# yassine-cherni/mujoco_ros2_simulation

Hardware: AMD Instinct MI355X
Metric: env-steps/sec (whole node), 7-DoF arm+lidar scene at 1/2/4/8 MI355X (higher is better)
Workload: dtype f32

## Files before the change

### include/mrs.h

```cpp
#ifndef MRS_H
#define MRS_H

#include "mrs_model.h"

#ifdef __cplusplus
extern "C" {
#endif

typedef struct mrs_model mrs_model;
typedef struct mrs_batch mrs_batch;

enum {
  MRS_OK = 0,
  MRS_ERR_INVALID = -1,
  MRS_ERR_LOAD = -2,
  MRS_ERR_DEVICE = -3,
  MRS_ERR_UNSUPPORTED = -4
};

enum {
  MRS_FIELD_QPOS = 0,
  MRS_FIELD_QVEL = 1,
  MRS_FIELD_CTRL = 2,
  MRS_FIELD_QFRC_APPLIED = 3,
// ... 101 lines not shown
int mrs_batch_get_contact_forces(mrs_batch* b, int env, int max, double* force);
float* mrs_batch_contact_wrench_device_ptr(mrs_batch* b);
int mrs_batch_get_contact_wrench(mrs_batch* b, double* host, int env0, int n);
enum {
  MRS_DYNOUT_QFRC_BIAS = 0,
  MRS_DYNOUT_MASS_MATRIX = 1,
  MRS_DYNOUT_SITE_JAC = 2,
  MRS_DYNOUT_SITE_POSE = 3,
  MRS_DYNOUT_COUNT = 4
};
#define MRS_MAX_JAC_SITES 16
int mrs_batch_set_jac_sites(mrs_batch* b, const int* site_ids, int n);
int mrs_batch_dyn_dim(const mrs_batch* b, int which);
float* mrs_batch_dyn_device_ptr(mrs_batch* b, int which);
int mrs_batch_get_dyn(mrs_batch* b, int which, double* host, int env0, int n);
int mrs_batch_get_efc(mrs_batch* b, int env, int max, int* type, double* J, double* R, double* aref,
                      double* force);
int mrs_batch_get_field_device(mrs_batch* b, int field, float* d_out, int env0, int n);
int mrs_batch_sync(mrs_batch* b);
double mrs_batch_last_kernel_ms(mrs_batch* b, int kind);
int mrs_batch_set_timing(mrs_batch* b, int mask);
int mrs_debug_phase_cycles(double* out, int n, int reset);
int mrs_debug_batch_layout(const mrs_batch* b, int* out, int n);
int mrs_debug_plan_layout(const mrs_model* m, int n_envs, int cu_count, int max_contacts, int* out, int n);
int mrs_debug_render_plan(const mrs_model* m, int cam, int n_frames, int max_lds, long long* out, int n);
int mrs_debug_ray_filter(const mrs_model* m, unsigned group_mask, int flags, int bodyexclude, int* out, int max);

#ifdef __cplusplus
}
#endif
#endif
```

### mujoco_ros2_simulation_amd/csrc/capi.cc

```cpp
#include <algorithm>
#include <cstring>
#include <memory>
#include <stdexcept>
#include <string>
#include <vector>

#include "../../include/mrs.h"
#include "hip/batch.h"
#include "mjcf/model.h"
#include "hip/rayfilter.h"
#include "hip/start_rows.h"
#include "mjcf/xml.h"

struct mrs_model {
  mrs::Model m;
};
struct mrs_batch {
  mrs::BatchImpl* impl = nullptr;
  const mrs_model* model = nullptr;
};

namespace {

thread_local std::string g_last_error;
// ... 532 lines not shown
  return ms;
}

int mrs_debug_phase_cycles(double* out, int n, int reset) {
  if (!out || n < 0) return MRS_ERR_INVALID;
  return mrs::phase_cycles(out, n, reset != 0);
}

int mrs_debug_batch_layout(const mrs_batch* b, int* out, int n) {
  if (!b || !out || n < 0) return MRS_ERR_INVALID;
  return mrs::batch_layout(b->impl, out, n);
}

int mrs_debug_plan_layout(const mrs_model* m, int n_envs, int cu_count, int max_contacts, int* out, int n) {
  int k = 0;
  const int rc = guarded([&] {
    if (!m || !out || n < 0) throw std::invalid_argument("null model or output");
    if (n_envs < 1) throw std::invalid_argument("n_envs must be positive");
    k = mrs::plan_layout(m->m, n_envs, cu_count, max_contacts, out, n);
  });
  return rc == MRS_OK ? k : rc;
}

int mrs_debug_render_plan(const mrs_model* m, int cam, int n_frames, int max_lds, long long* out, int n) {
  int k = 0;
  const int rc = guarded([&] {
    if (!m || !out || n < 0) throw std::invalid_argument("null model or output");
    if (n_frames < 1) throw std::invalid_argument("n_frames must be positive");
    if (max_lds < 0) throw std::invalid_argument("negative LDS limit");
    k = mrs::render_plan(m->m, cam, n_frames, max_lds, out, n);
  });
  return rc == MRS_OK ? k : rc;
}

int mrs_debug_ray_filter(const mrs_model* m, unsigned group_mask, int flags, int bodyexclude, int* out, int max) {
  int k = 0;
  const int rc = guarded([&] {
    if (!m) throw std::invalid_argument("null model");
    if (max < 0 || (max > 0 && !out)) throw std::invalid_argument("null output or negative capacity");
    mrs::check_ray_filter(m->m, flags, bodyexclude);
    const std::vector<mrs::RayGeom> list =
        mrs::build_ray_filter(m->m, group_mask, (flags & MRS_RAY_NO_STATIC) != 0, bodyexclude);
    k = static_cast<int>(list.size());
    for (int i = 0; i < k && i < max; ++i) out[i] = list[i].id;
  });
  return rc == MRS_OK ? k : rc;
// ... 4 lines not shown
```

### mujoco_ros2_simulation_amd/csrc/hip/batch.h

```cpp
#pragma once

#include <stdexcept>
#include <string>

namespace mrs {

struct Model;
struct BatchImpl;

struct DeviceError : std::runtime_error { using std::runtime_error::runtime_error; };
struct UnsupportedError : std::runtime_error { using std::runtime_error::runtime_error; };

BatchImpl* batch_create(const Model* model, int n_envs, int device, int max_contacts);
void batch_free(BatchImpl* b);
int batch_num_envs(const BatchImpl* b);
int batch_layout(const BatchImpl* b, int* out, int n);
int plan_layout(const Model& m, int n_envs, int cu_count, int max_contacts, int* out, int n);
void batch_set_stream(BatchImpl* b, void* stream);
void batch_reset(BatchImpl* b, int key, int env0, int n);
void batch_set_start_states(BatchImpl* b, const double* qpos, const double* qvel, int count);
void batch_set_start_states_device(BatchImpl* b, const float* d_qpos, const float* d_qvel, int count);
int batch_num_start_states(const BatchImpl* b);
void batch_reset_masked_device(BatchImpl* b, const unsigned char* d_mask, const int* d_key, int key);
void batch_reset_masked(BatchImpl* b, const unsigned char* mask, const int* keys, int key);
void batch_set(BatchImpl* b, int field, const double* host, int env0, int n);
void batch_get(BatchImpl* b, int field, double* host, int env0, int n);
void* batch_device_ptr(BatchImpl* b, int field);
void batch_set_act(BatchImpl* b, const double* host, int env0, int n);
void batch_get_act(BatchImpl* b, double* host, int env0, int n);
float* batch_act_device_ptr(BatchImpl* b);
void batch_set_mocap(BatchImpl* b, const double* pos, const double* quat, int env0, int n);
void batch_get_mocap(BatchImpl* b, double* pos, double* quat, int env0, int n);
float* batch_mocap_pos_device_ptr(BatchImpl* b);
float* batch_mocap_quat_device_ptr(BatchImpl* b);
int batch_param_dim(BatchImpl* b, int param);
void batch_set_param(BatchImpl* b, int param, const double* host, int env0, int n);
void batch_get_param(BatchImpl* b, int param, double* host, int env0, int n);
float* batch_param_device_ptr(BatchImpl* b, int param);
int batch_inertial_dim(BatchImpl* b, int which);
void batch_set_inertial(BatchImpl* b, const double* mass, const double* inertia, const double* armature, int env0, int n);
// ... 31 lines not shown
```

### mujoco_ros2_simulation_amd/csrc/hip/batch.hip

```cpp
#include <hip/hip_runtime.h>

#include <algorithm>
#include <cmath>
#include <cstdio>
#include <cstdlib>
#include <cstring>
#include <deque>
#include <initializer_list>
#include <stdexcept>
#include <string>
#include <thread>
#include <type_traits>
#include <utility>
#include <vector>

#include "../../../include/mrs.h"
#include "../mjcf/model.h"
#include "batch.h"
#include "batch_impl.h"
#include "devmodel.h"
#include "devtables.h"
#include "plan.h"
#include "lit.h"
#include "start_rows.h"
// ... 150 lines not shown
    a.bind(dalloc(b, static_cast<size_t>(b.n) * std::max(1, a.dim) * a.width()));
  }
}

void build_devmodel(BatchImpl& b, int max_con_req, const Overrides& o) {
  const Model& m = *b.model;
  const DevTables T = build_tables(m, max_con_req, o);
  int cus = 0;
  if (hipDeviceGetAttribute(&cus, hipDeviceAttributeMultiprocessorCount, b.device) != hipSuccess) cus = 0;
  const Plan p = choose_plan(m, T, b.n, cus, o);
  void* made[kArrCount];
  for (int id = 0; id < kArrCount; ++id) made[id] = env_array(b, id).ptr;
  b.dm = p.dm;
  for (int id = 0; id < kArrCount; ++id)
    if (made[id]) env_array(b, id).bind(made[id]);
  b.dblock_f = dalloc(b, T.f.size() * sizeof(float));
  b.dblock_i = dalloc(b, T.i.size() * sizeof(int));
  HIP_CHECK(hipMemcpyAsync(b.dblock_f, T.f.data(), T.f.size() * sizeof(float), hipMemcpyHostToDevice, b.stream));
  HIP_CHECK(hipMemcpyAsync(b.dblock_i, T.i.data(), T.i.size() * sizeof(int), hipMemcpyHostToDevice, b.stream));
  T.patch(b.dm, static_cast<const float*>(b.dblock_f), static_cast<const int*>(b.dblock_i));
  b.dm.rf_static = b.dm.rf_mode ? static_cast<float*>(dalloc(b, std::max(1, b.dm.nrf) * sizeof(float))) : nullptr;
  b.group = p.group; b.g16_one_wg = p.g16_one_wg; b.wpb16 = p.wpb16; b.helpers = p.helpers; b.ext = p.ext;
  b.pair_g1 = T.pair_g1; b.pair_g2 = T.pair_g2; b.pair_dim = T.pair_dim; b.pair_mu = T.pair_mu;
  b.d_dm = static_cast<DevModel*>(dalloc(b, sizeof(DevModel)));
  HIP_CHECK(hipMemcpyAsync(b.d_dm, &b.dm, sizeof(DevModel), hipMemcpyHostToDevice, b.stream));
  HIP_CHECK(hipStreamSynchronize(b.stream));
}

struct RowStage { double* host; std::vector<float> f; std::vector<int> i; };

void rows_to_device(BatchImpl& b, int env0, int n, std::initializer_list<std::pair<EnvArray, const double*>> parts) {
  HIP_CHECK(hipSetDevice(b.device));
  std::deque<RowStage> stage;
  bool queued = false;
  for (const auto& part : parts) {
    const EnvArray& a = part.first;
    const double* host = part.second;
    const size_t cnt = static_cast<size_t>(n) * std::max(0, a.dim);
    if (!host || cnt == 0) continue;
    const void* src = host;
    if (a.type == EnvArray::F32) {
      std::vector<float>& t = stage.emplace_back().f;
      t.resize(cnt);
      for (size_t k = 0; k < cnt; ++k) t[k] = static_cast<float>(host[k]);
      src = t.data();
    } else if (a.type == EnvArray::I32) {
// ... 204 lines not shown
  return b;
}

void batch_free(BatchImpl* b) {
  if (!b) return;
  (void)hipSetDevice(b->device);
  if (b->stream) (void)hipStreamSynchronize(b->stream);
  if (b->rstream) (void)hipStreamSynchronize(b->rstream);
  for (void* p : b->allocs) (void)hipFree(p);
  if (b->pool_qpos) (void)hipFree(b->pool_qpos);
  if (b->pool_qvel) (void)hipFree(b->pool_qvel);
  render_free(*b);
  for (int k = 0; k < 2; ++k) {
    if (b->ev0[k]) (void)hipEventDestroy(b->ev0[k]);
    if (b->ev1[k]) (void)hipEventDestroy(b->ev1[k]);
  }
  if (b->own_stream) (void)hipStreamDestroy(b->own_stream);
  delete b;
}

int batch_num_envs(const BatchImpl* b) { return b->n; }

int batch_layout(const BatchImpl* b, int* out, int n) {
  int v[19];
  plan_layout_values(b->dm, b->group, b->g16_one_wg, b->wpb16, b->helpers, v);
  v[16] = b->dm.cfrc_contact ? 1 : 0;
  v[17] = b->dm.dyn_mask;
  v[18] = b->dm.solve_fuse;
  int k = 0;
  for (; k < n && k < 19; ++k) out[k] = v[k];
  return k;
}

int plan_layout(const Model& m, int n_envs, int cu_count, int max_contacts, int* out, int n) {
  const Overrides o = read_overrides();
  const DevTables T = build_tables(m, max_contacts, o);
  const Plan p = choose_plan(m, T, n_envs, cu_count, o);
  int v[kPlanLayoutValues];
  plan_layout_values(p.dm, p.group, p.g16_one_wg, p.wpb16, p.helpers, v);
  int k = 0;
  for (; k < n && k < kPlanLayoutValues; ++k) out[k] = v[k];
  return k;
}

void batch_set_stream(BatchImpl* b, void* stream) {
  b->stream = stream ? static_cast<hipStream_t>(stream) : b->own_stream;
}

void batch_reset(BatchImpl* b, int key, int env0, int n) {
  const Model& m = *b->model;
  check_env_range(*b, env0, n);
  if (key >= m.nkey) throw std::invalid_argument("keyframe index out of range");
  b->ctrl_bound = nullptr;
// ... 505 lines not shown
```

### mujoco_ros2_simulation_amd/csrc/hip/batch_impl.h

```cpp
#pragma once

#include <hip/hip_runtime.h>

#include <deque>
#include <stdexcept>
#include <string>
#include <vector>

#include "../mjcf/model.h"
#include "batch.h"
#include "devmodel.h"
#include "rayfilter.h"
#include "start_rows.h"

namespace mrs {

#define HIP_CHECK(x)                                                                         \
  do {                                                                                       \
    hipError_t err_ = (x);                                                                   \
    if (err_ != hipSuccess)                                                                  \
      throw DeviceError(std::string(#x) + " failed: " + hipGetErrorString(err_));            \
  } while (0)

struct BatchImpl {
// ... 7 lines not shown
  DevModel* d_dm = nullptr;
  LdsLayout& L = dm.L;
  ScratchLayout& S = dm.S;
  DevState st{};
  const float* ctrl_bound = nullptr;
  StartRows start;
  std::vector<double> inr_host;
  float *tab_qpos = nullptr, *tab_qvel = nullptr, *tab_ctrl = nullptr, *tab_act = nullptr;
  float *tab_mpos = nullptr, *tab_mquat = nullptr;
  double* tab_time = nullptr;
  float *pool_qpos = nullptr, *pool_qvel = nullptr;
  int pool_n = 0, pool_cap = 0;
  unsigned char* mask_stage = nullptr;
  int* key_stage = nullptr;
  void* dblock_f = nullptr;
  void* dblock_i = nullptr;
  std::vector<void*> allocs;
  hipStream_t own_stream = nullptr, stream = nullptr;
  hipEvent_t ev0[2] = {nullptr, nullptr}, ev1[2] = {nullptr, nullptr};
  bool ev_valid[2] = {false, false};
  int timing = 2;
  std::vector<float> staging;
  std::vector<int> pair_g1, pair_g2;
  std::vector<int> pair_dim;
  std::vector<float> pair_mu;
  int dyn_asked = 0;
  hipStream_t rstream = nullptr;
  hipEvent_t snap_ev = nullptr, rend_ev = nullptr;
  bool rend_pending = false;
  float *snap_gpos = nullptr, *snap_gmat = nullptr, *snap_cpos = nullptr, *snap_cmat = nullptr;
  unsigned long long* rast_list = nullptr;
  int rast_frames = 0;
  int max_lds = 0;
  struct RayList { unsigned group_mask; bool no_static; int bodyexclude; RayGeom* d; int count; bool mesh; };
  std::deque<RayList> ray_lists;
  bool ext = false;
};

inline void* dalloc(BatchImpl& b, size_t bytes) {
  void* p = nullptr;
  HIP_CHECK(hipMalloc(&p, bytes ? bytes : 16));
  HIP_CHECK(hipMemsetAsync(p, 0, bytes ? bytes : 16, b.stream));
  b.allocs.push_back(p);
  return p;
}

// ... 8 lines not shown
```

### mujoco_ros2_simulation_amd/csrc/hip/devtables.h

```cpp
#pragma once

#include <algorithm>
#include <array>
#include <cmath>
#include <cstdlib>
#include <cstring>
#include <functional>
#include <stdexcept>
#include <string>
#include <vector>

#include "../../../include/mrs.h"
#include "../mjcf/model.h"
#include "batch.h"
#include "devmodel.h"
#include "renderplan.h"
#include "start_rows.h"

namespace mrs {

struct Overrides {
  int group = 0;
  int g16_wpb = 0;
  bool g16_one_wg = false;
  bool ray_helpers = true;
  bool no_fuse_ih = false;
  bool no_solve_fuse = false;
  bool no_ray_sweep = false;
  bool no_static_rays = false;
  bool no_static_frame = false;
  bool kin_twopass = false;
  int sparse_off = 0;
  int diag_skip = 0;
  bool sensors_every_step = false;
  bool no_multiccd = false;
  bool no_bvh = false;
  int bvh_leaf = 4;
  bool bvh_median = false;
  int spread = 0;
};

inline Overrides read_overrides() {
  auto set = [](const char* name) { return std::getenv(name) != nullptr; };
  auto num = [](const char* name, int absent) { const char* e = std::getenv(name); return e ? std::atoi(e) : absent; };
  Overrides o;
  o.group = num("MRS_GROUP", 0);
  o.g16_wpb = num("MRS_G16_WPB", 0);
  o.g16_one_wg = set("MRS_G16_ONE_WG");
  o.ray_helpers = num("MRS_RAY_HELPERS", 1) != 0;
  o.no_fuse_ih = set("MRS_NO_FUSE_IH");
  o.no_solve_fuse = set("MRS_NO_SOLVE_FUSE");
  o.no_ray_sweep = set("MRS_NO_RAY_SWEEP");
  o.no_static_rays = set("MRS_NO_STATIC_RAYS");
  o.no_static_frame = set("MRS_NO_STATIC_FRAME");
  o.kin_twopass = set("MRS_KIN_TWOPASS");
  o.sparse_off = num("MRS_SPARSE_OFF", 0) & 15;
  o.diag_skip = num("MRS_DIAG_SKIP", 0);
  o.sensors_every_step = num("MRS_SENSORS_EVERY_STEP", 0) != 0;
  o.no_multiccd = set("MRS_NO_MULTICCD");
  o.no_bvh = set("MRS_NO_BVH");
  o.bvh_leaf = std::max(1, std::min(64, num("MRS_BVH_LEAF", 4)));
  o.bvh_median = set("MRS_BVH_MEDIAN");
  o.spread = std::max(0, std::min(3, num("MRS_SPREAD", 0)));
  return o;
}

constexpr int kRlitHead = 12, kRlitLight = 24, kRlitMat = 12, kRlitTex = 16, kRlitMaxLights = 8;

template <class T>
struct Slot {
  CPtr<T> DevModel::*member;
  size_t off, len;
};

struct DevTables {
  DevModel dm{};
  std::vector<float> f;
  std::vector<int> i;
  std::vector<Slot<float>> fslot;
  std::vector<Slot<int>> islot;
  std::vector<int> pair_g1, pair_g2, pair_dim;
  std::vector<float> pair_mu;
  std::vector<int> rf;
  bool rf_fixed = false;

  void addf(CPtr<float> DevModel::*dst, const std::vector<double>& v) {
    fslot.push_back({dst, f.size(), v.size()});
    for (double x : v) f.push_back(static_cast<float>(x));
    while (f.size() % 4) f.push_back(0);
  }
  void addf(CPtr<float> DevModel::*dst, const std::vector<float>& v) {
    fslot.push_back({dst, f.size(), v.size()});
    f.insert(f.end(), v.begin(), v.end());
    while (f.size() % 4) f.push_back(0);
  }
  void addi(CPtr<int> DevModel::*dst, const std::vector<int>& v) {
    islot.push_back({dst, i.size(), v.size()});
    i.insert(i.end(), v.begin(), v.end());
    while (i.size() % 4) i.push_back(0);
  }
  const float* table(CPtr<float> DevModel::*member) const {
    for (const auto& s : fslot)
      if (s.member == member) return f.data() + s.off;
    throw std::logic_error("table not packed");
  }
// ... 295 lines not shown
    if (ta == MRS_GEOM_HFIELD || tb == MRS_GEOM_HFIELD)
      throw UnsupportedError("collision pair of geom types " + std::to_string(ta) + "/" + std::to_string(tb) +
                             " is not implemented (geoms " + std::to_string(g1) + "," + std::to_string(g2) + ")");
    p.g1.push_back(ga); p.g2.push_back(gb);
    p.dim.push_back(std::max(m.geom_condim[ga], m.geom_condim[gb]));
    p.margin.push_back(static_cast<float>(std::max(m.geom_margin[ga], m.geom_margin[gb])));
    p.gap.push_back(static_cast<float>(std::max(m.geom_gap[ga], m.geom_gap[gb])));
    double s1 = m.geom_solmix[ga], s2 = m.geom_solmix[gb], mix;
    if (s1 >= 1e-15 && s2 >= 1e-15) mix = s1 / (s1 + s2);
    else if (s1 < 1e-15 && s2 < 1e-15) mix = 0.5;
    else mix = s1 < 1e-15 ? 0 : 1;
    for (int i = 0; i < 3; ++i)
      p.fric.push_back(static_cast<float>(std::max(m.geom_friction[3 * ga + i], m.geom_friction[3 * gb + i])));
    for (int i = 0; i < 2; ++i)
      p.solref.push_back(static_cast<float>(mix * m.geom_solref[2 * ga + i] + (1 - mix) * m.geom_solref[2 * gb + i]));
    for (int i = 0; i < 5; ++i)
      p.solimp.push_back(static_cast<float>(mix * m.geom_solimp[5 * ga + i] + (1 - mix) * m.geom_solimp[5 * gb + i]));
  }
  d.npair = static_cast<int>(p.g1.size());
  d.npair_explicit = static_cast<int>(m.expair_geom1.size());
  return p;
}

struct EqTables {
  std::vector<int> type, obj1, obj2;
  std::vector<double> solref, solimp, data;
};
inline EqTables equality_tables(const Model& m, DevModel& d) {
  EqTables e;
  d.neq = d.neq_rows = 0;
  if (!(m.disableflags & (MRS_DSBL_EQUALITY | MRS_DSBL_CONSTRAINT)))
    for (size_t q = 0; q < m.eq_type.size(); ++q) {
      if (!m.eq_active0[q]) continue;
      e.type.push_back(m.eq_type[q]); e.obj1.push_back(m.eq_obj1id[q]); e.obj2.push_back(m.eq_obj2id[q]);
      e.solref.insert(e.solref.end(), &m.eq_solref[2 * q], &m.eq_solref[2 * q] + 2);
      e.solimp.insert(e.solimp.end(), &m.eq_solimp[5 * q], &m.eq_solimp[5 * q] + 5);
      e.data.insert(e.data.end(), &m.eq_data[MRS_NEQDATA * q], &m.eq_data[MRS_NEQDATA * q] + MRS_NEQDATA);
      d.neq_rows += m.eq_type[q] == MRS_EQ_CONNECT ? 3 : (m.eq_type[q] == MRS_EQ_WELD ? 6 : 1);
    }
  d.neq = static_cast<int>(e.type.size());
  return e;
}

struct TendonTables {
  std::vector<int> adr, num, wrap_qadr, wrap_dof, fric, lim, sp_ten, sp_adr, sp_num, sp_of;
  std::vector<double> coef, J, prm;
// ... 533 lines not shown
    if (d.rf_static_frame) {
      double R[9], p[3];
      body_world(m, m.site_bodyid[site], R, p);
      const double d0[3] = {dir[0], dir[1], dir[2]}, o0[3] = {org[0], org[1], org[2]};
      for (int i = 0; i < 3; ++i) {
        dir[i] = R[3 * i] * d0[0] + R[3 * i + 1] * d0[1] + R[3 * i + 2] * d0[2];
        org[i] = p[i] + R[3 * i] * o0[0] + R[3 * i + 1] * o0[1] + R[3 * i + 2] * o0[2];
      }
    }
    rfray.insert(rfray.end(), {static_cast<float>(dir[0]), static_cast<float>(dir[1]), static_cast<float>(dir[2]),
                               int_bits(m.sensor_adr[rf[k]]), int_bits(m.site_bodyid[site]),
                               static_cast<float>(org[0]), static_cast<float>(org[1]), static_cast<float>(org[2])});
  }
  return rfray;
}

inline DevTables build_tables(const Model& m, int max_con_req, const Overrides& o) {
  if (m.nv > 64) throw UnsupportedError("nv > 64 is not supported by the one-wave-per-env kernel");
  DevTables T;
  DevModel& d = T.dm;
  using D = DevModel;
  model_counts(m, o, d);
  const TreeLists trees = tree_lists(m, o, d);
  const PairTables pairs = collision_pairs(m, d);
  T.pair_g1 = pairs.g1;
  T.pair_g2 = pairs.g2;
  T.pair_dim = pairs.dim;
  T.pair_mu.resize(pairs.g1.size());
  for (size_t q = 0; q < pairs.g1.size(); ++q) T.pair_mu[q] = pairs.fric[3 * q];
  const EqTables eq = equality_tables(m, d);
  const TendonTables ten = tendon_tables(m, d);
  d.xrows = d.neq + d.nten_fric + d.nten_lim;
  const KinTrees kt = kinematic_trees(m, pairs, d);
  const RowLists rows = row_lists(m, pairs, max_con_req, d);
  const ActTables act = actuator_tables(m, d);

  T.addi(&D::body_parentid, m.body_parentid); T.addi(&D::body_rootid, m.body_rootid);
  T.addi(&D::body_jntnum, m.body_jntnum); T.addi(&D::body_jntadr, m.body_jntadr);
  T.addi(&D::body_dofnum, m.body_dofnum); T.addi(&D::body_dofadr, m.body_dofadr);
  T.addi(&D::body_subtree_end, trees.subtree_end); T.addi(&D::level_adr, trees.level_adr);
  T.addi(&D::level_num, trees.level_num); T.addi(&D::level_body, trees.level_body); T.addi(&D::jump, trees.jump);
  T.addf(&D::body_pos, m.body_pos); T.addf(&D::body_quat, m.body_quat); T.addf(&D::body_ipos, m.body_ipos);
  T.addf(&D::body_iquat, m.body_iquat); T.addf(&D::body_mass, m.body_mass);
  T.addf(&D::body_subtreemass, m.body_subtreemass); T.addf(&D::body_inertia, m.body_inertia);
  T.addf(&D::body_gravcomp, m.body_gravcomp); T.addf(&D::body_invweight0, m.body_invweight0);
  T.addi(&D::jnt_type, m.jnt_type); T.addi(&D::jnt_qposadr, m.jnt_qposadr); T.addi(&D::jnt_dofadr, m.jnt_dofadr);
  T.addi(&D::jnt_bodyid, m.jnt_bodyid); T.addi(&D::jnt_actfrclimited, m.jnt_actfrclimited);
  T.addf(&D::jnt_pos, m.jnt_pos); T.addf(&D::jnt_axis, m.jnt_axis); T.addf(&D::jnt_stiffness, m.jnt_stiffness);
  T.addf(&D::jnt_range, m.jnt_range); T.addf(&D::jnt_margin, m.jnt_margin); T.addf(&D::jnt_solref, m.jnt_solref);
  T.addf(&D::jnt_solimp, m.jnt_solimp); T.addf(&D::jnt_actfrcrange, m.jnt_actfrcrange);
  T.addi(&D::dof_bodyid, m.dof_bodyid); T.addi(&D::dof_jntid, m.dof_jntid);
  T.addf(&D::dof_armature, m.dof_armature); T.addf(&D::dof_damping, m.dof_damping);
  T.addf(&D::dof_frictionloss, m.dof_frictionloss); T.addf(&D::dof_solref, m.dof_solref);
  T.addf(&D::dof_solimp, m.dof_solimp); T.addf(&D::dof_invweight0, m.dof_invweight0);
  T.addf(&D::qpos0, m.qpos0); T.addf(&D::qpos_spring, m.qpos_spring);
  T.addi(&D::Mpair, trees.Mpair);
  T.addi(&D::body_tree, kt.body_tree); T.addi(&D::dof_tree, kt.dof_tree); T.addi(&D::tree_dofadr, kt.dofadr);
// ... 78 lines not shown
```

### mujoco_ros2_simulation_amd/csrc/hip/plan.h

```cpp
#pragma once

#include <algorithm>
#include <cmath>
#include <vector>

#include "devtables.h"

namespace mrs {

inline LdsLayout lds_layout(const Model& m, const DevModel& d, bool blocked, bool want_lh) {
  LdsLayout L{};
  int off = 0;
  auto take = [&](int n) { int o = off; off += n; off = (off + 3) & ~3; return o; };
  const int nb = m.nbody, nj = std::max(1, m.njnt), nv = std::max(1, m.nv), ng = std::max(1, m.ngeom);
  L.xpos = take(3 * nb); L.xquat = take(4 * nb); L.xmat = take(9 * nb); L.xipos = take(3 * nb);
  L.xanchor = take(3 * nj); L.xaxis = take(3 * nj); L.gxpos = take(3 * ng); L.gxmat = take(9 * ng);
  L.scom = take(3 * nb); L.cinert = take(10 * nb); L.crb = d.acc_sens ? take(10 * nb) : 0; L.cdof = take(6 * nv);
  L.cdofdot = take(6 * nv); L.cvel = take(6 * nb); L.cacc = take(6 * nb); L.cfrc = take(6 * nb);
  if (!d.acc_sens) L.crb = L.cacc;
  const int msize = blocked ? std::max(1, d.nMblk) : nv * nv;
  L.M = take(msize); L.L = take(msize); L.qpos = take(std::max(1, m.nq)); L.qvel = take(nv);
  L.ctrl = take(std::max(1, m.nu)); L.qfrc_applied = take(nv); L.qacc_ws = take(nv); L.qfrc_bias = take(nv);
  L.qfrc_passive = take(nv); L.qfrc_act = take(nv); L.qfrc_smooth = take(nv); L.qacc_smooth = take(nv);
  L.qacc = take(nv + 1); L.qfrc_con = take(nv + 1);
// ... 35 lines not shown
  d.shr_kjnt = d.shr_kbody + 25 * m.nbody;
  d.shr_kgeom = d.shr_kjnt + 13 * m.njnt;
  d.shr_flag = d.shr_kgeom + 9 * m.ngeom;
  d.shr_total = d.shr_flag + 4;
  return d;
}

inline ScratchLayout scratch_layout(const Model& m, const DevModel& d, bool blocked) {
  ScratchLayout S{};
  int off = 0;
  auto take = [&](int n) { int o = off; off += n; off = (off + 3) & ~3; return o; };
  const int nv = std::max(1, m.nv), ne = std::max(1, d.max_efc);
  const int dn = blocked && m.solver == MRS_SOL_PGS && m.cone != MRS_CONE_ELLIPTIC && d.xrows == 0 ? 0 : ne;
  S.efc_J = take(dn * nv); S.efc_MJ = take(dn * nv); S.efc_type = take(ne); S.efc_pos = take(ne);
  S.efc_margin = take(ne); S.efc_floss = take(ne); S.efc_R = take(dn); S.efc_aref = take(dn);
  S.efc_b = take(dn); S.efc_f = take(ne); S.efc_ARii = take(dn); S.con = take(kConRec * std::max(1, d.max_con));
  S.efc_rec = take(blocked ? ne * (2 * d.pipe_w + 12) : 0);
  S.efc_rowof = take(blocked ? ne : 0);
  S.efc_item = take(blocked ? ne : 0);
  S.efc_fq = take(blocked ? ne : 0);
  S.efc_hdr = take(blocked ? 24 * ne : 0);
  S.efc_quad = take(blocked ? 64 : 0);
  S.efc_fd = take(m.cone == MRS_CONE_ELLIPTIC && m.solver == MRS_SOL_PGS ? 2 * ne : 0);
  S.stage = take(d.npair > 0 ? 64 * kMaxPairCon * 7 : 0);
  S.efc_n = take(1);
  S.sens = take(std::max(1, m.nsensordata));
  S.xfrc = take(1);
  S.total = off;
  return S;
}

struct Plan {
  int group = 64;
  int g16_one_wg = 0;
  int wpb16 = WavesPerBlock<16>::value;
  int helpers = 0;
  bool ext = false;
  bool want_lh = false;
  DevModel dm{};
};

inline void fit_ray_sweep(const Model& m, const DevTables& T, DevModel& d) {
  const float *rgeom = T.table(&DevModel::rgeom), *rfray = T.table(&DevModel::rfray), *rfblk = T.table(&DevModel::rfblk);
  bool ok = true;
  for (int i = 0; i < d.nrgeom; ++i)
    if (!((d.rf_static_mask >> i) & 1u) && bits_int(rgeom[8 * i + 1]) == MRS_GEOM_MESH) ok = false;
  const int adr0 = m.sensor_adr[T.rf[0]];
// ... 74 lines not shown
  d = shared_layout(m, d);
  auto lds_bytes = [&](const DevModel& s, int g) {
    return (static_cast<size_t>(d.L.total) * envs_per_block(g) + (g == 64 ? s.shr_act : s.shr_total)) * sizeof(float);
  };
  for (int g : {32, 16})
    if (m.nv <= g && lds_bytes(d, g) <= 80 * 1024) p.group = g;
  if (p.group > 16 && m.nv <= 16) {
    DevModel without = d;
    without.rf_common = 0;
    without = shared_layout(m, without);
    if (d.rf_common && lds_bytes(without, 16) <= 80 * 1024) {
      p.group = 16;
      d = without;
    }
    if (p.group > 16 && lds_bytes(d, 16) <= 160 * 1024 && o.g16_one_wg) { p.group = 16; p.g16_one_wg = 1; }
  }
  if ((o.group == 8 || o.group == 16 || o.group == 32 || o.group == 64) && m.nv <= o.group) p.group = o.group;
  const long waves = (static_cast<long>(n_envs) * 16 + 63) / 64;
  if (p.group == 16 && !p.g16_one_wg) {
    if (cu_count > 0 && waves < 4L * cu_count) p.wpb16 = 1;
    if (o.g16_wpb == 1 || o.g16_wpb == 2 || o.g16_wpb == 4)
      p.wpb16 = std::min(o.g16_wpb, static_cast<int>(WavesPerBlock<16>::value));
  }
  p.ext = d.nrgeom > 32 && d.nrf > 0;
  for (size_t q = 0; q < T.pair_g1.size() && !p.ext; ++q) {
    const int t1 = m.geom_type[T.pair_g1[q]], t2 = m.geom_type[T.pair_g2[q]];
    auto conv = [](int t) { return t == MRS_GEOM_ELLIPSOID || t == MRS_GEOM_CYLINDER || t == MRS_GEOM_MESH; };
    if (t1 != MRS_GEOM_PLANE && t2 != MRS_GEOM_PLANE && (conv(t1) || conv(t2))) p.ext = true;
  }
  const bool fit = cu_count <= 0 || waves <= 2L * cu_count;
  p.helpers = o.ray_helpers && fit && p.group == 16 && p.wpb16 == 1 && !p.ext && d.nrf > 0 && d.nrgeom <= 32 &&
              m.integrator != MRS_INT_RK4 && !(m.disableflags & MRS_DSBL_SENSOR) ? 1 : 0;
  p.want_lh = p.helpers && m.integrator != MRS_INT_IMPLICIT;
  bool flim = false;
  for (int a = 0; a < m.nu; ++a) flim |= m.actuator_forcelimited[a] != 0;
  d.fuse_ih = p.group == 16 && !p.helpers && m.integrator == MRS_INT_IMPLICITFAST && !flim && m.nv <= 16 &&
              !o.no_fuse_ih ? 1 : 0;
  if (d.fuse_ih && m.solver != MRS_SOL_PGS && !p.want_lh) {
    const size_t with_lh = static_cast<size_t>(lds_layout(m, d, false, true).total) * envs_per_block(p.group, p.wpb16) + d.shr_total;
    if (with_lh * sizeof(float) > 160 * 1024) d.fuse_ih = 0;
    else p.want_lh = true;
  }
  d.solve_fuse = p.group == 16 && m.solver == MRS_SOL_PGS && !p.helpers && !o.no_solve_fuse ? 1 : 0;
  if (d.rf_mode == 2 && d.rf_common && d.rf_static_frame && d.nrgeom <= 32 && (p.group == 16 || p.group == 32) &&
      !p.helpers && d.nrf >= 3 && (d.nrf + p.group - 1) / p.group <= 32 && !o.no_ray_sweep)
    fit_ray_sweep(m, T, d);
  d.blocked = p.group == 64 ? 1 : 0;
  if (d.blocked) d.shr_total = d.shr_act;
  d.L = lds_layout(m, d, d.blocked != 0, p.want_lh);
  d.lds_tenJ = lds_tenj(m, d, d.L);
  d.shr_off = d.L.total * envs_per_block(p.group, p.wpb16);
  if ((static_cast<size_t>(d.shr_off) + d.shr_total) * sizeof(float) > 160 * 1024)
// ... 15 lines not shown
```

### mujoco_ros2_simulation_amd/sim.py

```python
from __future__ import annotations

import ctypes as C
import os
from pathlib import Path

import numpy as np

_PKG = Path(__file__).resolve().parent
LIB_PATH = Path(os.environ["MRS_LIB"]) if os.environ.get("MRS_LIB") else _PKG / "libmrs.so"

GEOM_PLANE, GEOM_HFIELD, GEOM_SPHERE, GEOM_CAPSULE, GEOM_ELLIPSOID, GEOM_CYLINDER, GEOM_BOX, GEOM_MESH = range(8)
JNT_FREE, JNT_BALL, JNT_SLIDE, JNT_HINGE = range(4)
OBJ_BODY, OBJ_JOINT, OBJ_GEOM, OBJ_SITE, OBJ_CAMERA, OBJ_ACTUATOR, OBJ_SENSOR = 1, 3, 5, 6, 7, 19, 20
OBJ_TENDON = 18
SENS_ACCELEROMETER, SENS_GYRO, SENS_FORCE, SENS_TORQUE, SENS_RANGEFINDER = 1, 3, 4, 5, 7
SENS_JOINTPOS, SENS_JOINTVEL, SENS_ACTUATORFRC, SENS_FRAMEPOS, SENS_FRAMEQUAT = 9, 10, 15, 25, 26
SENS_TOUCH, SENS_VELOCIMETER, SENS_FRAMEXAXIS, SENS_FRAMEYAXIS, SENS_FRAMEZAXIS = 0, 2, 27, 28, 29
SENS_FRAMELINVEL, SENS_FRAMEANGVEL, SENS_FRAMELINACC, SENS_SUBTREECOM, SENS_SUBTREELINVEL = 30, 31, 32, 34, 35
SENS_TENDONPOS, SENS_TENDONVEL = 11, 12
BIAS_NONE, BIAS_AFFINE = 0, 1
RESTATE_NEWTON_REFINE, RESTATE_PGS_ELLIPTIC_BLOCK, RESTATE_NO_MPR_POLISH, RESTATE_NO_MULTICCD = 1, 2, 4, 8
(FIELD_QPOS, FIELD_QVEL, FIELD_CTRL, FIELD_QFRC_APPLIED, FIELD_QACC_WARMSTART, FIELD_QACC,
 FIELD_QFRC_ACTUATOR, FIELD_SENSORDATA, FIELD_TIME, FIELD_WARNING, FIELD_NCON, FIELD_SOLVER_NITER,
 FIELD_XFRC_APPLIED) = range(13)
# ... 231 lines not shown
            L.mrs_batch_contact_wrench_device_ptr.restype = C.c_void_p
            L.mrs_batch_contact_wrench_device_ptr.argtypes = [C.c_void_p]
            L.mrs_batch_get_contact_wrench.argtypes = [C.c_void_p, C.c_void_p, C.c_int, C.c_int]
        if hasattr(L, "mrs_batch_get_dyn"):
            L.mrs_batch_set_jac_sites.argtypes = [C.c_void_p, C.c_void_p, C.c_int]
            L.mrs_batch_dyn_dim.argtypes = [C.c_void_p, C.c_int]
            L.mrs_batch_dyn_device_ptr.restype = C.c_void_p
            L.mrs_batch_dyn_device_ptr.argtypes = [C.c_void_p, C.c_int]
            L.mrs_batch_get_dyn.argtypes = [C.c_void_p, C.c_int, C.c_void_p, C.c_int, C.c_int]
        if hasattr(L, "mrs_batch_ray"):
            L.mrs_batch_ray_device.argtypes = [C.c_void_p, C.c_void_p, C.c_void_p, C.c_int, C.c_int, C.c_int, C.c_int,
                                               C.c_uint, C.c_int, C.c_void_p, C.c_void_p]
            L.mrs_batch_ray.argtypes = [C.c_void_p, C.c_void_p, C.c_void_p, C.c_int, C.c_int, C.c_int, C.c_int,
                                        C.c_uint, C.c_int, C.c_void_p, C.c_void_p, C.c_int, C.c_int]
            L.mrs_debug_ray_filter.argtypes = [C.c_void_p, C.c_uint, C.c_int, C.c_int, C.c_void_p, C.c_int]
        L.mrs_batch_get_field_device.argtypes = [C.c_void_p, C.c_int, C.c_void_p, C.c_int, C.c_int]
        L.mrs_batch_last_kernel_ms.restype = C.c_double
        L.mrs_batch_last_kernel_ms.argtypes = [C.c_void_p, C.c_int]
        L.mrs_debug_phase_cycles.argtypes = [C.c_void_p, C.c_int, C.c_int]
        L.mrs_debug_batch_layout.argtypes = [C.c_void_p, C.c_void_p, C.c_int]
        L.mrs_debug_plan_layout.argtypes = [C.c_void_p, C.c_int, C.c_int, C.c_int, C.c_void_p, C.c_int]
        if hasattr(L, "mrs_debug_render_plan"):
            L.mrs_debug_render_plan.argtypes = [C.c_void_p, C.c_int, C.c_int, C.c_int, C.c_void_p, C.c_int]
        _lib = L
    return _lib


PHASES = ["kinematics", "com_pos", "make_M", "cholesky", "com_vel", "rne", "smooth_forces", "collision",
          "constraints", "sensors", "integrate", "checks", "sensors.level1", "sensors.setup", "sensors.geoms",
          "constraints.rows", "constraints.records", "constraints.warmstart", "constraints.pgs",
          "collision.narrow", "collision.out", "constraints.delassus", "records.jac", "records.solve",
          "records.rows"]


def phase_cycles(reset: bool = False) -> dict | None:
    out = np.zeros(len(PHASES))
    n = lib().mrs_debug_phase_cycles(out.ctypes.data_as(C.c_void_p), len(PHASES), int(reset))
    if n <= 0:
        return None
    return dict(zip(PHASES, out[:n].tolist()))


def _check(rc: int) -> None:
    if rc != MRS_OK:
        raise MrsError(rc, lib().mrs_last_error().decode())

# ... 83 lines not shown
    def handle(self) -> int:
        return self._h

    def __del__(self):
        if getattr(self, "_h", None) and _lib is not None:
            _lib.mrs_model_free(self._h)
            self._h = None


_FIELD_DIM = {
    FIELD_QPOS: (1, "nq"), FIELD_QVEL: (1, "nv"), FIELD_CTRL: (1, "nu"), FIELD_QFRC_APPLIED: (1, "nv"),
    FIELD_QACC_WARMSTART: (1, "nv"), FIELD_QACC: (1, "nv"), FIELD_QFRC_ACTUATOR: (1, "nv"),
    FIELD_SENSORDATA: (1, "nsensordata"), FIELD_TIME: (1, None), FIELD_WARNING: (4, None), FIELD_NCON: (1, None),
    FIELD_SOLVER_NITER: (1, None), FIELD_XFRC_APPLIED: (6, "nbody"),
}


LAYOUT_KEYS = ["group", "lds_floats", "scratch_floats", "blocked", "pipe_w", "max_efc", "max_con", "ntree",
               "shared_floats", "rf_common", "one_workgroup_per_cu", "waves_per_workgroup", "helper_waves",
               "fused_integrator_factor", "ray_sweep", "sensors_every_step"]
LAYOUT_OUTPUT_KEYS = ["contact_wrench"]
LAYOUT_DYN_KEYS = ["dyn_outputs"]
LAYOUT_SOLVE_KEYS = ["solve_fuse"]


def plan_layout(model: "Model", n_envs: int, cu_count: int, max_contacts: int = 0) -> dict:
    out = np.zeros(len(LAYOUT_KEYS), dtype=np.int32)
    k = lib().mrs_debug_plan_layout(model.handle, n_envs, cu_count, max_contacts, out.ctypes.data, len(out))
    if k < 0:
        raise MrsError(k, lib().mrs_last_error().decode())
    return dict(zip(LAYOUT_KEYS[:k], out[:k].tolist()))


RENDER_KERNELS = ["binned", "frame", "tile"]


def render_plan(model: "Model", cam: int, n_frames: int, max_lds: int) -> dict:
    out = np.zeros(7, dtype=np.int64)
    k = lib().mrs_debug_render_plan(model.handle, cam, n_frames, max_lds, out.ctypes.data, len(out))
    if k < 0:
        raise MrsError(k, lib().mrs_last_error().decode())
    v = out.tolist()
    return {"kernel": RENDER_KERNELS[v[0]], "mesh": bool(v[1]), "band_lds": v[2], "chunk": v[3], "per_frame": v[4],
            "grid": (v[5], v[6])}


def ray_filter(model: "Model", group_mask: int = 0, include_static: bool = True, bodyexclude: int = -1) -> np.ndarray:
    out = np.zeros(max(1, model.ngeom), dtype=np.int32)
    k = lib().mrs_debug_ray_filter(model.handle, group_mask, 0 if include_static else RAY_NO_STATIC, bodyexclude,
                                   out.ctypes.data, model.ngeom)
    if k < 0:
        raise MrsError(k, lib().mrs_last_error().decode())
    return out[:k].copy()

# ... 144 lines not shown

    def reset_where(self, mask, keys=None, key: int = -1) -> None:
        mask = np.asarray(mask)
        if mask.shape != (self.n,):
            raise ValueError(f"mask must have shape ({self.n},), not {mask.shape}")
        if mask.dtype not in (np.bool_, np.uint8):
            raise ValueError(f"mask must be bool or uint8, not {mask.dtype}")
        mask = np.ascontiguousarray(mask).view(np.uint8)
        if keys is not None:
            keys = np.asarray(keys)
            if keys.shape != (self.n,):
                raise ValueError(f"keys must have shape ({self.n},), not {keys.shape}")
            if keys.dtype != np.int32:
                raise ValueError(f"keys must be int32, not {keys.dtype}")
            keys = np.ascontiguousarray(keys)
        _check(lib().mrs_batch_reset_masked(self._h, mask.ctypes.data, keys.ctypes.data if keys is not None else None,
                                             key))

    def reset_where_device(self, mask_ptr: int, keys_ptr: int = 0, key: int = -1) -> None:
        _check(lib().mrs_batch_reset_masked_device(self._h, C.c_void_p(mask_ptr) if mask_ptr else None,
                                                    C.c_void_p(keys_ptr) if keys_ptr else None, key))

    def layout(self) -> dict:
        keys = LAYOUT_KEYS + LAYOUT_OUTPUT_KEYS + LAYOUT_DYN_KEYS + LAYOUT_SOLVE_KEYS
        out = np.zeros(len(keys), dtype=np.int32)
        k = lib().mrs_debug_batch_layout(self._h, out.ctypes.data, len(keys))
        return dict(zip(keys[:k], out[:k].tolist()))

    def step(self, n_steps: int = 1) -> None:
        _check(lib().mrs_batch_step(self._h, n_steps))

    def forward(self) -> None:
        _check(lib().mrs_batch_forward(self._h))

    def sync(self) -> None:
        _check(lib().mrs_batch_sync(self._h))

    def device_ptr(self, field: int) -> int:
        return lib().mrs_batch_device_ptr(self._h, field)

    def set_ctrl_device(self, ptr: int) -> None:
        _check(lib().mrs_batch_set_ctrl_device(self._h, C.c_void_p(ptr)))

    def bind_ctrl_device(self, ptr: int | None) -> None:
        _check(lib().mrs_batch_bind_ctrl_device(self._h, C.c_void_p(ptr) if ptr else None))

    def set_stream(self, stream_ptr: int | None) -> None:
# ... 137 lines not shown
```

Before: 292.0 million.

## Prune collision pairs that can never touch using static reach bounds

At model build time, computes a conservative reach sphere for each geom from the hinge/ball joint chain and drops collision pairs (including plane pairs) whose bounding spheres can never overlap. Fewer pairs are walked by the narrowphase each step, while row/tree sizing and the convex-pair layout decision still use the full pair list so buffer sizes are unchanged. A debug API and env-var opt-out are added. The risk is a pruning bound that is not actually conservative, which would miss real contacts.

```diff
diff --git a/include/mrs.h b/include/mrs.h
--- a/include/mrs.h
+++ b/include/mrs.h
@@ -147,6 +147,7 @@
 int mrs_batch_set_timing(mrs_batch* b, int mask);
 int mrs_debug_phase_cycles(double* out, int n, int reset);
 int mrs_debug_batch_layout(const mrs_batch* b, int* out, int n);
+int mrs_debug_pairs(const mrs_model* m, int* geom, int max, int* pruned);
 int mrs_debug_plan_layout(const mrs_model* m, int n_envs, int cu_count, int max_contacts, int* out, int n);
 int mrs_debug_render_plan(const mrs_model* m, int cam, int n_frames, int max_lds, long long* out, int n);
 int mrs_debug_ray_filter(const mrs_model* m, unsigned group_mask, int flags, int bodyexclude, int* out, int max);
diff --git a/mujoco_ros2_simulation_amd/csrc/capi.cc b/mujoco_ros2_simulation_amd/csrc/capi.cc
--- a/mujoco_ros2_simulation_amd/csrc/capi.cc
+++ b/mujoco_ros2_simulation_amd/csrc/capi.cc
@@ -578,6 +578,16 @@
   return rc == MRS_OK ? k : rc;
 }
 
+int mrs_debug_pairs(const mrs_model* m, int* geom, int max, int* pruned) {
+  int k = 0;
+  const int rc = guarded([&] {
+    if (!m) throw std::invalid_argument("null model");
+    if (max < 0 || (max > 0 && !geom)) throw std::invalid_argument("null output or negative capacity");
+    k = mrs::walked_pairs(m->m, geom, max, pruned);
+  });
+  return rc == MRS_OK ? k : rc;
+}
+
 int mrs_debug_render_plan(const mrs_model* m, int cam, int n_frames, int max_lds, long long* out, int n) {
   int k = 0;
   const int rc = guarded([&] {
diff --git a/mujoco_ros2_simulation_amd/csrc/hip/batch.h b/mujoco_ros2_simulation_amd/csrc/hip/batch.h
--- a/mujoco_ros2_simulation_amd/csrc/hip/batch.h
+++ b/mujoco_ros2_simulation_amd/csrc/hip/batch.h
@@ -16,6 +16,7 @@
 int batch_num_envs(const BatchImpl* b);
 int batch_layout(const BatchImpl* b, int* out, int n);
 int plan_layout(const Model& m, int n_envs, int cu_count, int max_contacts, int* out, int n);
+int walked_pairs(const Model& m, int* geom, int max, int* pruned);
 void batch_set_stream(BatchImpl* b, void* stream);
 void batch_reset(BatchImpl* b, int key, int env0, int n);
 void batch_set_start_states(BatchImpl* b, const double* qpos, const double* qvel, int count);
diff --git a/mujoco_ros2_simulation_amd/csrc/hip/batch.hip b/mujoco_ros2_simulation_amd/csrc/hip/batch.hip
--- a/mujoco_ros2_simulation_amd/csrc/hip/batch.hip
+++ b/mujoco_ros2_simulation_amd/csrc/hip/batch.hip
@@ -196,6 +196,7 @@
   b.dm.rf_static = b.dm.rf_mode ? static_cast<float*>(dalloc(b, std::max(1, b.dm.nrf) * sizeof(float))) : nullptr;
   b.group = p.group; b.g16_one_wg = p.g16_one_wg; b.wpb16 = p.wpb16; b.helpers = p.helpers; b.ext = p.ext;
   b.pair_g1 = T.pair_g1; b.pair_g2 = T.pair_g2; b.pair_dim = T.pair_dim; b.pair_mu = T.pair_mu;
+  b.pairs_pruned = T.pairs_pruned;
   b.d_dm = static_cast<DevModel*>(dalloc(b, sizeof(DevModel)));
   HIP_CHECK(hipMemcpyAsync(b.d_dm, &b.dm, sizeof(DevModel), hipMemcpyHostToDevice, b.stream));
   HIP_CHECK(hipStreamSynchronize(b.stream));
@@ -446,13 +447,23 @@
 int batch_num_envs(const BatchImpl* b) { return b->n; }
 
 int batch_layout(const BatchImpl* b, int* out, int n) {
-  int v[19];
+  int v[21];
   plan_layout_values(b->dm, b->group, b->g16_one_wg, b->wpb16, b->helpers, v);
   v[16] = b->dm.cfrc_contact ? 1 : 0;
   v[17] = b->dm.dyn_mask;
   v[18] = b->dm.solve_fuse;
+  v[19] = b->dm.npair;
+  v[20] = b->pairs_pruned;
   int k = 0;
-  for (; k < n && k < 19; ++k) out[k] = v[k];
+  for (; k < n && k < 21; ++k) out[k] = v[k];
+  return k;
+}
+
+int walked_pairs(const Model& m, int* geom, int max, int* pruned) {
+  const DevTables T = build_tables(m, 0, read_overrides());
+  const int k = static_cast<int>(T.pair_g1.size());
+  for (int q = 0; q < k && q < max; ++q) { geom[2 * q] = T.pair_g1[q]; geom[2 * q + 1] = T.pair_g2[q]; }
+  if (pruned) *pruned = T.pairs_pruned;
   return k;
 }
 
diff --git a/mujoco_ros2_simulation_amd/csrc/hip/batch_impl.h b/mujoco_ros2_simulation_amd/csrc/hip/batch_impl.h
--- a/mujoco_ros2_simulation_amd/csrc/hip/batch_impl.h
+++ b/mujoco_ros2_simulation_amd/csrc/hip/batch_impl.h
@@ -53,6 +53,7 @@
   int timing = 2;
   std::vector<float> staging;
   std::vector<int> pair_g1, pair_g2;
+  int pairs_pruned = 0;
   std::vector<int> pair_dim;
   std::vector<float> pair_mu;
   int dyn_asked = 0;
diff --git a/mujoco_ros2_simulation_amd/csrc/hip/devtables.h b/mujoco_ros2_simulation_amd/csrc/hip/devtables.h
--- a/mujoco_ros2_simulation_amd/csrc/hip/devtables.h
+++ b/mujoco_ros2_simulation_amd/csrc/hip/devtables.h
@@ -27,6 +27,7 @@
   bool no_fuse_ih = false;
   bool no_solve_fuse = false;
   bool no_ray_sweep = false;
+  bool no_pair_prune = false;
   bool no_static_rays = false;
   bool no_static_frame = false;
   bool kin_twopass = false;
@@ -51,6 +52,7 @@
   o.no_fuse_ih = set("MRS_NO_FUSE_IH");
   o.no_solve_fuse = set("MRS_NO_SOLVE_FUSE");
   o.no_ray_sweep = set("MRS_NO_RAY_SWEEP");
+  o.no_pair_prune = set("MRS_NO_PAIR_PRUNE");
   o.no_static_rays = set("MRS_NO_STATIC_RAYS");
   o.no_static_frame = set("MRS_NO_STATIC_FRAME");
   o.kin_twopass = set("MRS_KIN_TWOPASS");
@@ -81,6 +83,8 @@
   std::vector<Slot<int>> islot;
   std::vector<int> pair_g1, pair_g2, pair_dim;
   std::vector<float> pair_mu;
+  int pairs_pruned = 0;
+  bool convex_pairs = false;
   std::vector<int> rf;
   bool rf_fixed = false;
 
@@ -422,6 +426,92 @@
   return p;
 }
 
+struct Reach {
+  bool bounded = true, fixed = true;
+  double c[3] = {0, 0, 0}, last[3] = {0, 0, 0}, rho = 0;
+};
+inline std::vector<Reach> geom_reach(const Model& m) {
+  auto point = [&](int body, const double* local, double out[3]) {
+    double R[9], p[3];
+    body_world(m, body, R, p);
+    for (int i = 0; i < 3; ++i) out[i] = p[i] + R[3 * i] * local[0] + R[3 * i + 1] * local[1] + R[3 * i + 2] * local[2];
+  };
+  auto dist = [](const double a[3], const double b[3]) {
+    return std::sqrt((a[0] - b[0]) * (a[0] - b[0]) + (a[1] - b[1]) * (a[1] - b[1]) + (a[2] - b[2]) * (a[2] - b[2]));
+  };
+  std::vector<Reach> body(m.nbody);
+  for (int b = 1; b < m.nbody; ++b) {
+    Reach r = body[m.body_parentid[b]];
+    if (m.body_mocapid[b] >= 0 || m.body_jntnum[b] > 1) r.bounded = false;
+    if (r.bounded && m.body_jntnum[b] == 1) {
+      const int j = m.body_jntadr[b];
+      if (m.jnt_type[j] != MRS_JNT_HINGE && m.jnt_type[j] != MRS_JNT_BALL) r.bounded = false;
+      else {
+        double a[3];
+        point(b, &m.jnt_pos[3 * j], a);
+        if (r.fixed) std::copy(a, a + 3, r.c);
+        else r.rho += dist(a, r.last);
+        std::copy(a, a + 3, r.last);
+        r.fixed = false;
+      }
+    }
+    body[b] = r;
+  }
+  std::vector<Reach> geom(m.ngeom);
+  for (int g = 0; g < m.ngeom; ++g) {
+    Reach r = body[m.geom_bodyid[g]];
+    if (r.bounded) {
+      double x[3];
+      point(m.geom_bodyid[g], &m.geom_pos[3 * g], x);
+      if (r.fixed) std::copy(x, x + 3, r.c);
+      else r.rho += dist(x, r.last);
+    }
+    geom[g] = r;
+  }
+  return geom;
+}
+
+inline bool never_touch(const Model& m, const std::vector<Reach>& reach, int ga, int gb, double margin) {
+  const auto slack = [](double r) { return r * (1 + 1e-4) + 1e-4; };
+  const bool pa = m.geom_type[ga] == MRS_GEOM_PLANE, pb = m.geom_type[gb] == MRS_GEOM_PLANE;
+  if (pa || pb) {
+    const int pl = pa ? ga : gb, g = pa ? gb : ga;
+    if (pa && pb) return false;
+    if (!fixed_in_world(m, m.geom_bodyid[pl]) || !reach[g].bounded) return false;
+    double R[9], p[3], Rg[9], n[3], o[3], q[4];
+    body_world(m, m.geom_bodyid[pl], R, p);
+    const double* gq = &m.geom_quat[4 * pl];
+    const double qn = std::sqrt(gq[0] * gq[0] + gq[1] * gq[1] + gq[2] * gq[2] + gq[3] * gq[3]);
+    for (int i = 0; i < 4; ++i) q[i] = gq[i] / qn;
+    quat_to_mat(q, Rg);
+    for (int i = 0; i < 3; ++i) {
+      n[i] = R[3 * i] * Rg[2] + R[3 * i + 1] * Rg[5] + R[3 * i + 2] * Rg[8];
+      o[i] = p[i] + R[3 * i] * m.geom_pos[3 * pl] + R[3 * i + 1] * m.geom_pos[3 * pl + 1] + R[3 * i + 2] * m.geom_pos[3 * pl + 2];
+    }
+    const double h = n[0] * (reach[g].c[0] - o[0]) + n[1] * (reach[g].c[1] - o[1]) + n[2] * (reach[g].c[2] - o[2]);
+    return h > slack(reach[g].rho + m.geom_rbound[g] + margin);
+  }
+  if (!reach[ga].bounded || !reach[gb].bounded) return false;
+  const double* a = reach[ga].c;
+  const double* b = reach[gb].c;
+  const double dc = std::sqrt((a[0] - b[0]) * (a[0] - b[0]) + (a[1] - b[1]) * (a[1] - b[1]) + (a[2] - b[2]) * (a[2] - b[2]));
+  return dc > slack(reach[ga].rho + reach[gb].rho + m.geom_rbound[ga] + m.geom_rbound[gb] + margin);
+}
+inline PairTables prune_pairs(const Model& m, const PairTables& all, const Overrides& o) {
+  if (o.no_pair_prune) return all;
+  const std::vector<Reach> reach = geom_reach(m);
+  PairTables p;
+  for (size_t q = 0; q < all.g1.size(); ++q) {
+    if (q >= m.expair_geom1.size() && never_touch(m, reach, all.g1[q], all.g2[q], all.margin[q])) continue;
+    p.g1.push_back(all.g1[q]); p.g2.push_back(all.g2[q]); p.dim.push_back(all.dim[q]);
+    p.margin.push_back(all.margin[q]); p.gap.push_back(all.gap[q]);
+    p.fric.insert(p.fric.end(), &all.fric[3 * q], &all.fric[3 * q] + 3);
+    p.solref.insert(p.solref.end(), &all.solref[2 * q], &all.solref[2 * q] + 2);
+    p.solimp.insert(p.solimp.end(), &all.solimp[5 * q], &all.solimp[5 * q] + 5);
+  }
+  return p;
+}
+
 struct EqTables {
   std::vector<int> type, obj1, obj2;
   std::vector<double> solref, solimp, data;
@@ -1001,7 +1091,14 @@
   using D = DevModel;
   model_counts(m, o, d);
   const TreeLists trees = tree_lists(m, o, d);
-  const PairTables pairs = collision_pairs(m, d);
+  const PairTables all_pairs = collision_pairs(m, d);
+  const PairTables pairs = prune_pairs(m, all_pairs, o);
+  T.pairs_pruned = static_cast<int>(all_pairs.g1.size() - pairs.g1.size());
+  for (size_t q = 0; q < all_pairs.g1.size(); ++q) {
+    const int t1 = m.geom_type[all_pairs.g1[q]], t2 = m.geom_type[all_pairs.g2[q]];
+    auto conv = [](int t) { return t == MRS_GEOM_ELLIPSOID || t == MRS_GEOM_CYLINDER || t == MRS_GEOM_MESH; };
+    if (t1 != MRS_GEOM_PLANE && t2 != MRS_GEOM_PLANE && (conv(t1) || conv(t2))) T.convex_pairs = true;
+  }
   T.pair_g1 = pairs.g1;
   T.pair_g2 = pairs.g2;
   T.pair_dim = pairs.dim;
@@ -1010,8 +1107,9 @@
   const EqTables eq = equality_tables(m, d);
   const TendonTables ten = tendon_tables(m, d);
   d.xrows = d.neq + d.nten_fric + d.nten_lim;
-  const KinTrees kt = kinematic_trees(m, pairs, d);
-  const RowLists rows = row_lists(m, pairs, max_con_req, d);
+  const KinTrees kt = kinematic_trees(m, all_pairs, d);
+  const RowLists rows = row_lists(m, all_pairs, max_con_req, d);
+  d.npair = static_cast<int>(pairs.g1.size());
   const ActTables act = actuator_tables(m, d);
 
   T.addi(&D::body_parentid, m.body_parentid); T.addi(&D::body_rootid, m.body_rootid);
diff --git a/mujoco_ros2_simulation_amd/csrc/hip/plan.h b/mujoco_ros2_simulation_amd/csrc/hip/plan.h
--- a/mujoco_ros2_simulation_amd/csrc/hip/plan.h
+++ b/mujoco_ros2_simulation_amd/csrc/hip/plan.h
@@ -81,7 +81,7 @@
   S.efc_hdr = take(blocked ? 24 * ne : 0);
   S.efc_quad = take(blocked ? 64 : 0);
   S.efc_fd = take(m.cone == MRS_CONE_ELLIPTIC && m.solver == MRS_SOL_PGS ? 2 * ne : 0);
-  S.stage = take(d.npair > 0 ? 64 * kMaxPairCon * 7 : 0);
+  S.stage = take(d.max_con > 0 ? 64 * kMaxPairCon * 7 : 0);
   S.efc_n = take(1);
   S.sens = take(std::max(1, m.nsensordata));
   S.xfrc = take(1);
@@ -202,12 +202,7 @@
     if (o.g16_wpb == 1 || o.g16_wpb == 2 || o.g16_wpb == 4)
       p.wpb16 = std::min(o.g16_wpb, static_cast<int>(WavesPerBlock<16>::value));
   }
-  p.ext = d.nrgeom > 32 && d.nrf > 0;
-  for (size_t q = 0; q < T.pair_g1.size() && !p.ext; ++q) {
-    const int t1 = m.geom_type[T.pair_g1[q]], t2 = m.geom_type[T.pair_g2[q]];
-    auto conv = [](int t) { return t == MRS_GEOM_ELLIPSOID || t == MRS_GEOM_CYLINDER || t == MRS_GEOM_MESH; };
-    if (t1 != MRS_GEOM_PLANE && t2 != MRS_GEOM_PLANE && (conv(t1) || conv(t2))) p.ext = true;
-  }
+  p.ext = (d.nrgeom > 32 && d.nrf > 0) || T.convex_pairs;
   const bool fit = cu_count <= 0 || waves <= 2L * cu_count;
   p.helpers = o.ray_helpers && fit && p.group == 16 && p.wpb16 == 1 && !p.ext && d.nrf > 0 && d.nrgeom <= 32 &&
               m.integrator != MRS_INT_RK4 && !(m.disableflags & MRS_DSBL_SENSOR) ? 1 : 0;
diff --git a/mujoco_ros2_simulation_amd/sim.py b/mujoco_ros2_simulation_amd/sim.py
--- a/mujoco_ros2_simulation_amd/sim.py
+++ b/mujoco_ros2_simulation_amd/sim.py
@@ -277,6 +277,8 @@
         L.mrs_debug_plan_layout.argtypes = [C.c_void_p, C.c_int, C.c_int, C.c_int, C.c_void_p, C.c_int]
         if hasattr(L, "mrs_debug_render_plan"):
             L.mrs_debug_render_plan.argtypes = [C.c_void_p, C.c_int, C.c_int, C.c_int, C.c_void_p, C.c_int]
+        if hasattr(L, "mrs_debug_pairs"):
+            L.mrs_debug_pairs.argtypes = [C.c_void_p, C.c_void_p, C.c_int, C.c_void_p]
         _lib = L
     return _lib
 
@@ -406,6 +408,7 @@
 LAYOUT_OUTPUT_KEYS = ["contact_wrench"]
 LAYOUT_DYN_KEYS = ["dyn_outputs"]
 LAYOUT_SOLVE_KEYS = ["solve_fuse"]
+LAYOUT_PAIR_KEYS = ["pairs", "pairs_pruned"]
 
 
 def plan_layout(model: "Model", n_envs: int, cu_count: int, max_contacts: int = 0) -> dict:
@@ -414,6 +417,16 @@
     if k < 0:
         raise MrsError(k, lib().mrs_last_error().decode())
     return dict(zip(LAYOUT_KEYS[:k], out[:k].tolist()))
+
+
+def walked_pairs(model: "Model") -> tuple[np.ndarray, int]:
+    pruned = C.c_int(0)
+    k = lib().mrs_debug_pairs(model.handle, None, 0, C.byref(pruned))
+    if k < 0:
+        raise MrsError(k, lib().mrs_last_error().decode())
+    out = np.zeros((k, 2), dtype=np.int32)
+    lib().mrs_debug_pairs(model.handle, out.ctypes.data if k else None, k, None)
+    return out, pruned.value
 
 
 RENDER_KERNELS = ["binned", "frame", "tile"]
@@ -604,7 +617,7 @@
                                                     C.c_void_p(keys_ptr) if keys_ptr else None, key))
 
     def layout(self) -> dict:
-        keys = LAYOUT_KEYS + LAYOUT_OUTPUT_KEYS + LAYOUT_DYN_KEYS + LAYOUT_SOLVE_KEYS
+        keys = LAYOUT_KEYS + LAYOUT_OUTPUT_KEYS + LAYOUT_DYN_KEYS + LAYOUT_SOLVE_KEYS + LAYOUT_PAIR_KEYS
         out = np.zeros(len(keys), dtype=np.int32)
         k = lib().mrs_debug_batch_layout(self._h, out.ctypes.data, len(keys))
         return dict(zip(keys[:k], out[:k].tolist()))
```

After: 304.0 million (median of 6 runs). +4.1%, better.
